# Dao-AILab/flash-attention

Measured on AMD Instinct MI355X. Metric: attention_fwd_tflops, higher is better.
Workload: dtype bf16; 1 GPU; BASELINE config 3: B=4 H=32 S=4096 D=128 bf16 causal, forward (flash_attn_func path, fa_fwd via C ABI); batch=4, heads=32, seqlen=4096, head_dim=128, causal=True, parallelism=replicas x1

## Files before the change

flash-attention_amd/csrc/fa_fwd_w64.hip:

```cpp
#include <cstdio>
#include <cstdlib>
#include <type_traits>

#include "fa_device.h"
#include "fa_kernel_params.h"
#include "fa_launch.h"
#include "fa_fwd_w64_regs.h"
#define FA_W64_CLOB FA_W64_ACC_CLOBBERS
#include "fa_w64_asm.h"


#define FA_W64_AH 3
#define FA_W64_KDMA_G0 0
#define FA_W64_KDMA_GS 2
#define FA_W64_VDMA_G0 1
#define FA_W64_VDMA_GS 2

namespace fa {

template <int D> FA_DEVINL constexpr int k_swz_w(int row) { return D == 128 ? (row & 15) : ((row >> 1) & 7); }
template <int D> FA_DEVINL constexpr int v_swz_w(int row) { return D == 128 ? (row & 3) : ((row >> 1) & 1); }

#define FA_W64_MFMA(E_) (std::is_same<E_, __bf16>::value ? "v_mfma_f32_32x32x16_bf16" : "v_mfma_f32_32x32x16_f16")
constexpr int W64_Q_BASE = 128;
template <typename E, int F> FA_DEVINL void mfma_s_first(f32x16& d, u32x4 a, const f32x16& c) {
  if constexpr (std::is_same<E, __bf16>::value)
    asm volatile("v_mfma_f32_32x32x16_bf16 %0, %1, a[%c3:%c4], %2" : "=&v"(d) : "v"(a), "v"(c), "i"(W64_Q_BASE + 4 * F), "i"(W64_Q_BASE + 4 * F + 3) : FA_W64_ACC_CLOBBERS);
  else
    asm volatile("v_mfma_f32_32x32x16_f16 %0, %1, a[%c3:%c4], %2" : "=&v"(d) : "v"(a), "v"(c), "i"(W64_Q_BASE + 4 * F), "i"(W64_Q_BASE + 4 * F + 3) : FA_W64_ACC_CLOBBERS);
}
template <typename E, int F> FA_DEVINL void mfma_s_acc(f32x16& d, u32x4 a) {
  if constexpr (std::is_same<E, __bf16>::value)
    asm volatile("v_mfma_f32_32x32x16_bf16 %0, %1, a[%c2:%c3], %0" : "+v"(d) : "v"(a), "i"(W64_Q_BASE + 4 * F), "i"(W64_Q_BASE + 4 * F + 3) : FA_W64_ACC_CLOBBERS);
  else
    asm volatile("v_mfma_f32_32x32x16_f16 %0, %1, a[%c2:%c3], %0" : "+v"(d) : "v"(a), "i"(W64_Q_BASE + 4 * F), "i"(W64_Q_BASE + 4 * F + 3) : FA_W64_ACC_CLOBBERS);
}
template <typename E, int T> FA_DEVINL void mfma_o_acc(u32x4 a, u32x4 b) {
  if constexpr (std::is_same<E, __bf16>::value)
    asm volatile("v_mfma_f32_32x32x16_bf16 a[%c2:%c3], %0, %1, a[%c2:%c3]" : : "v"(a), "v"(b), "i"(16 * T), "i"(16 * T + 15) : FA_W64_ACC_CLOBBERS);
  else
    asm volatile("v_mfma_f32_32x32x16_f16 a[%c2:%c3], %0, %1, a[%c2:%c3]" : : "v"(a), "v"(b), "i"(16 * T), "i"(16 * T + 15) : FA_W64_ACC_CLOBBERS);
}
template <typename E, int D, int FEAT = 0, bool PAGED = false>
__global__ void __launch_bounds__(256, 1) fa_fwd_w64_kernel(const FwdK p) {
  constexpr bool ALIBI = FEAT == FEAT_ALIBI;
  static_assert(!PAGED || FEAT == 0, "the paged variant serves plain attention");
  constexpr bool SOFTCAP = FEAT == FEAT_CAP;
  constexpr bool DROP = FEAT == FEAT_DROP;
  constexpr bool DESC = ALIBI;
  static_assert(FEAT == 0 || FEAT == FEAT_ALIBI || FEAT == FEAT_CAP || FEAT == FEAT_DROP, "feature variants of this schedule: none, causal ALiBi, softcap, dropout");
  using T = ElemTraits<E>;
  using V8 = typename T::v8;
  constexpr int NW = 4, QB = 2, BM = NW * 64, BN = 64, CPR = D / 8;
  constexpr int ROW_BYTES = D * 2;
  constexpr int TILE_BYTES = BN * ROW_BYTES;
  constexpr int KS = D / 16;
  constexpr int DB = D / 32;
  static_assert(D == 64 || D == 128, "head dims built natively: 64, 128");
  constexpr float kLn2 = 0.6931471805599453f;

  extern __shared__ __attribute__((aligned(16))) char smem[];
  char FA_LDS* lds = (char FA_LDS*)smem;
  constexpr int STAGE_BYTES = BM * (ROW_BYTES + 16);
  constexpr int Q_OFF = (4 * TILE_BYTES > STAGE_BYTES ? 4 * TILE_BYTES : STAGE_BYTES + 1023) / 1024 * 1024;

  const int tid = threadIdx.x;
  const int lane = tid & 63;
  const int wave = __builtin_amdgcn_readfirstlane(tid >> 6);
  const int hi = lane >> 5, qi = lane & 31;

  const int d_row = lane / CPR, d_pc = lane % CPR;
  constexpr int RPD = 1024 / ROW_BYTES;

  struct Blk { int b, h, m_block, sq, sk; int64_t q_row0, k_row0, q_boff, k_boff, v_boff, o_boff; };
  const int n_virtual = p.persist_total > 0 ? p.persist_total : (int)gridDim.x;
  const bool snake = p.persist_total > 0 && p.wr >= 0 && p.unit_size > 1 && ((int)(gridDim.x / 8) % p.unit_size) == 0;
  auto decode_id = [&](int vb, int round, Blk& k) __attribute__((always_inline)) -> bool {
    if (vb >= n_virtual) return false;
    if (p.work_list) {
      if (!work_list_item(p.work_list, vb, p.h, p.h_k, k.b, k.h, k.m_block)) return false;
    } else {
      int bid = vb;
      if (snake && (round & 1)) {
        const int slot = vb / 8, item = slot % p.unit_size;
        bid = vb + 8 * (p.unit_size - 1 - 2 * item);
      }
      const int w = xcd_interleave(bid, p.n_units, p.unit_size, p.unit_hpx);
      if (w < 0) return false;
      const int bh = w / p.nmb;
      const int mbr = w - bh * p.nmb;
      k.m_block = (p.wr >= 0) ? (p.nmb - 1 - mbr) : mbr;
      k.b = bh / p.h;
      k.h = bh - k.b * p.h;
    }
    return true;
  };
  auto fill_blk = [&](Blk& k) __attribute__((always_inline)) -> bool {
    k.sq = p.sq; k.sk = p.sk; k.q_row0 = 0; k.k_row0 = 0;
    const int bkv = p.kv_batch_idx ? p.kv_batch_idx[k.b] : k.b;
    k.q_boff = (int64_t)k.b * p.q_bs; k.k_boff = (int64_t)bkv * p.k_bs; k.v_boff = (int64_t)bkv * p.v_bs; k.o_boff = (int64_t)k.b * p.o_bs;
    if (p.cu_q) { const int c0 = p.cu_q[k.b]; k.sq = p.cu_q[k.b + 1] - c0; k.q_row0 = c0; k.q_boff = 0; k.o_boff = 0; }
    if (p.seqused_q) k.sq = min(k.sq, p.seqused_q[k.b]);
    if (p.cu_k) { const int c0 = p.cu_k[k.b]; k.sk = p.cu_k[k.b + 1] - c0; k.k_row0 = c0; k.k_boff = 0; k.v_boff = 0; }
    if (p.seqused_k) k.sk = min(p.seqused_k[k.b] + p.seqused_add, (p.cu_k && !PAGED) ? k.sk : p.sk);
    if (p.leftpad_k) {
      const int lp = p.leftpad_k[k.b];
      k.sk = max(0, k.sk - lp);
      k.k_row0 += lp;
    }
    if constexpr (PAGED) { k.k_boff = 0; k.v_boff = 0; k.k_row0 = 0; }
    return k.m_block * BM < k.sq;
  };
  constexpr int QDMA = (BM * ROW_BYTES) / 1024 / NW;
  auto q_srd_of = [&](const Blk& k) __attribute__((always_inline)) {
    const E* base = (const E*)p.q + k.q_boff + (k.q_row0 + (int64_t)k.m_block * BM) * p.q_rs + (int64_t)k.h * p.q_hs;
    const int rows = min(BM, k.sq - k.m_block * BM);
    const unsigned long long a = (unsigned long long)base;
// ... 87 lines not shown
    const unsigned long long a = (unsigned long long)base;
    const unsigned lo = __builtin_amdgcn_readfirstlane((unsigned)a);
    const unsigned hi16 = __builtin_amdgcn_readfirstlane((unsigned)(a >> 32)) & 0xffffu;
    const unsigned long long bytes = sk > 0 ? ((unsigned long long)(sk - 1) * (unsigned long long)row_stride + D) * 2ull : 0ull;
    const unsigned nrec = __builtin_amdgcn_readfirstlane((unsigned)(bytes > 0xffffffffull ? 0xffffffffull : bytes));
    u32x4 s = {lo, hi16, nrec, 0x00020000u};
    return s;
  };
  const u32x4 k_srd = make_srd(kp, p.k_rs), v_srd = make_srd(vp, p.v_rs);
  const u32x4 null_srd = {k_srd[0], k_srd[1], 0u, k_srd[3]};
  const int pg_tpp = __builtin_amdgcn_readfirstlane(PAGED ? p.page_size / BN : 1);
  const int pg_last = __builtin_amdgcn_readfirstlane(sk > 0 ? (sk - 1) / max(p.page_size, 1) : 0);
  const int* __restrict__ pg_table = p.block_table + (PAGED ? (int64_t)__builtin_amdgcn_readfirstlane(b) * p.block_table_bs : 0);
  auto page_entry = [&](int page) __attribute__((always_inline)) {
    const int pc = min(max(page, 0), pg_last);
    return __builtin_amdgcn_readfirstlane(pg_table[pc]);
  };
  const unsigned pg_bytes_k = (unsigned)__builtin_amdgcn_readfirstlane((int)(unsigned)(p.k_bs * 2)), pg_bytes_v = (unsigned)__builtin_amdgcn_readfirstlane((int)(unsigned)(p.v_bs * 2));
  const unsigned tl_bytes_k = (unsigned)__builtin_amdgcn_readfirstlane((int)(unsigned)(BN * p.k_rs * 2)), tl_bytes_v = (unsigned)__builtin_amdgcn_readfirstlane((int)(unsigned)(BN * p.v_rs * 2));
  auto uniform64 = [](const void* ptr) __attribute__((always_inline)) {
    const unsigned long long a = (unsigned long long)ptr;
    const unsigned lo = (unsigned)__builtin_amdgcn_readfirstlane((int)(unsigned)a), hi = (unsigned)__builtin_amdgcn_readfirstlane((int)(unsigned)(a >> 32));
    return ((unsigned long long)hi << 32) | (unsigned long long)lo;
  };
  const unsigned long long pg_base_k = uniform64(kp), pg_base_v = uniform64(vp);
  auto tile_srd = [&](auto isvc, int blk, int tin, int n) __attribute__((always_inline)) {
    constexpr bool ISV = decltype(isvc)::value != 0;
    const unsigned rs = (unsigned)(ISV ? p.v_rs : p.k_rs);
    const int rows = (n >= 0) ? min(BN, sk - n * BN) : 0;
    const unsigned long long a = (ISV ? pg_base_v : pg_base_k) + (unsigned long long)(unsigned)blk * (unsigned long long)(ISV ? pg_bytes_v : pg_bytes_k) + (unsigned long long)((unsigned)tin * (ISV ? tl_bytes_v : tl_bytes_k));
    const unsigned nrec = rows > 0 ? ((unsigned)(rows - 1) * rs + (unsigned)D) * 2u : 0u;
    u32x4 sd = {(unsigned)a, (unsigned)(a >> 32) & 0xffffu, nrec, 0x00020000u};
    return sd;
  };
  auto dma_pieces = [&](const u32x4& srd, const unsigned (&vo)[DPW], unsigned lds_dst) __attribute__((always_inline)) {
    unsigned keep;
    const unsigned dst = __builtin_amdgcn_readfirstlane(lds_dst);
    if constexpr (DPW == 4) {
      asm volatile("s_mov_b32 %0, m0\n\ts_mov_b32 m0, %5\n\ts_nop 0\n\t"
                   "buffer_load_dwordx4 %1, %6, 0 offen lds\n\t"
                   "buffer_load_dwordx4 %2, %6, 0 offen offset:1024 lds\n\t"
                   "buffer_load_dwordx4 %3, %6, 0 offen offset:2048 lds\n\t"
                   "buffer_load_dwordx4 %4, %6, 0 offen offset:3072 lds\n\t"
                   "s_mov_b32 m0, %0"
                   : "=&s"(keep) : "v"(vo[0]), "v"(vo[1]), "v"(vo[2]), "v"(vo[3]), "s"(dst), "s"(srd) : "memory");
    } else {
      asm volatile("s_mov_b32 %0, m0\n\ts_mov_b32 m0, %3\n\ts_nop 0\n\t"
                   "buffer_load_dwordx4 %1, %4, 0 offen lds\n\t"
                   "buffer_load_dwordx4 %2, %4, 0 offen offset:1024 lds\n\t"
                   "s_mov_b32 m0, %0"
                   : "=&s"(keep) : "v"(vo[0]), "v"(vo[DPW - 1]), "s"(dst), "s"(srd) : "memory");
    }
  };
  auto dma_tile = [&](auto isvc, int buf, int t) __attribute__((always_inline)) {
    constexpr bool ISV = decltype(isvc)::value != 0;
    const bool real = t >= 0 && t < n_tiles;
    const int64_t rs = ISV ? p.v_rs : p.k_rs;
    const unsigned lds_dst = (unsigned)((ISV ? 2 + buf : buf) * TILE_BYTES + wave * DPW * 1024);
    if constexpr (PAGED) {
      const int n = n_min + t, page = max(n, 0) / pg_tpp;
      const u32x4 sd = real ? tile_srd(isvc, page_entry(page), max(n, 0) - page * pg_tpp, n) : null_srd;
      dma_pieces(sd, ISV ? voff_l : koff_l, lds_dst);
      return;
    }
    const unsigned toff = real ? (unsigned)(n_min + t) * (unsigned)(BN * 2) * (unsigned)rs : 0u;
    unsigned vo[DPW];
#pragma unroll
    for (int i = 0; i < DPW; ++i) vo[i] = (ISV ? voff_l[i] : koff_l[i]) + toff;
    dma_pieces(real ? (ISV ? v_srd : k_srd) : null_srd, vo, lds_dst);
  };

  __syncthreads();
  if (q_in_lds != vb) dma_q(q_srd_of(blk));
  if (n_tiles > 0) dma_tile(ICw<0>{}, 0, tile_of(0));
  if (q_in_lds != vb) {
    if (n_tiles > 0) { if constexpr (DPW == 4) asm volatile("s_waitcnt vmcnt(4)" ::: "memory"); else asm volatile("s_waitcnt vmcnt(2)" ::: "memory"); }
    else lds_dma_wait_all();
  }
  {
    const float cq = SOFTCAP ? p.scale * 2.885390081777927f / p.softcap : p.scale_log2;
    u32x4 qraw[QB][KS];
#pragma unroll
    for (int qb = 0; qb < QB; ++qb)
#pragma unroll
      for (int ks = 0; ks < KS; ++ks) {
        const int qbase = Q_OFF + (wave * 64 + qb * 32 + qi) * ROW_BYTES + ((hi ^ k_swz_w<D>(qi)) << 4);
        qraw[qb][ks] = *(const u32x4 FA_LDS*)(unsigned long)(unsigned)(qbase ^ (ks << 5));
      }
    auto load_q = [&](auto qbc, auto ksc) __attribute__((always_inline)) {
      constexpr int qb = decltype(qbc)::value, ks = decltype(ksc)::value;
      const V8 raw = bitcast_u32x4<V8>(qraw[qb][ks]);
      V8 sc;
#pragma unroll
      for (int j = 0; j < 8; j += 2) {
        typedef __attribute__((ext_vector_type(2))) float f32x2;
        f32x2 pr = {(float)raw[j], (float)raw[j + 1]};
        pr *= f32x2{cq, cq};
        sc[j] = (E)pr[0]; sc[j + 1] = (E)pr[1];
      }
      acc_write_frag<W64_Q_BASE + 4 * (qb * KS + ks)>(__builtin_bit_cast(u32x4, sc));
    };
    auto load_q_all = [&](auto qbc) __attribute__((always_inline)) {
      load_q(qbc, ICw<0>{}); load_q(qbc, ICw<1>{}); load_q(qbc, ICw<2>{}); load_q(qbc, ICw<3>{});
      if constexpr (KS == 8) { load_q(qbc, ICw<4>{}); load_q(qbc, ICw<5>{}); load_q(qbc, ICw<6>{}); load_q(qbc, ICw<7>{}); }
    };
    load_q_all(ICw<0>{});
    if (n_tiles > 0) dma_tile(ICw<1>{}, 1, -1);
    load_q_all(ICw<1>{});
  }
  lds_dma_wait_all();
  __syncthreads();
  u32x4 qn_srd = null_srd;
  int qn_done = QDMA, qn_per_iter = QDMA;
  {
    q_in_lds = -1;
    if (nxt_id_ok && fill_blk(nxt)) {
      asm volatile("s_waitcnt lgkmcnt(0)" ::: "memory");
      qn_srd = q_srd_of(nxt); qn_done = 0;
      qn_per_iter = n_tiles >= QDMA ? 1 : n_tiles >= QDMA / 2 ? 2 : n_tiles >= QDMA / 4 ? 4 : QDMA;
      if (n_tiles == 0) { dma_q(qn_srd); lds_dma_wait_all(); qn_done = QDMA; }
      q_in_lds = vb + (int)gridDim.x;
    }
  }
  auto q_trickle = [&]() __attribute__((always_inline)) {
    if (qn_done < QDMA) {
#pragma unroll 1
      for (int j = 0; j < qn_per_iter; ++j) dma_q_piece(qn_srd, qn_done + j);
      qn_done += qn_per_iter;
    }
  };

  const int kbase = qi * ROW_BYTES + ((hi ^ k_swz_w<D>(qi)) << 4);
  const int tr_i = lane & 15, tr_half = (lane >> 4) & 1;
  const int tr_rr = tr_i >> 2, tr_cc = tr_i & 3;
  const int vbase = (4 * hi + tr_rr) * ROW_BYTES + (v_swz_w<D>(tr_rr) << 6) + tr_half * 32 + tr_cc * 8;
  int ka[KS], va[DB];
#pragma unroll
  for (int ks = 0; ks < KS; ++ks) ka[ks] = kbase ^ (ks << 5);
#pragma unroll
  for (int db = 0; db < DB; ++db) va[db] = vbase ^ (db << 6);

  {
    u32x4 zf = {0u, 0u, 0u, 0u};
    asm volatile("" : "+v"(zf));
    acc_zero_tuples_mfma<0>(zf, std::make_integer_sequence<int, 2 * DB>{});
  }
  float m_run[QB], l_run[QB][2], o_lag[QB];
  float thr_l[QB];
  float capc = 0.f, cap_m2c = 0.f, capoff[QB] = {0.f, 0.f};
  if constexpr (SOFTCAP) {
    capc = __builtin_bit_cast(float, __builtin_amdgcn_readfirstlane(__builtin_bit_cast(int, p.softcap * 1.4426950408889634f)));
    cap_m2c = -2.f * capc;
    capoff[0] = capc; capoff[1] = capc;
  }
  unsigned drop_kr[7] = {0u, 0u, 0u, 0u, 0u, 0u, 0u}, drop_thr = 255u, drop_row[QB] = {0u, 0u};
  if constexpr (DROP) {
    const unsigned k0_ = (unsigned)__builtin_amdgcn_readfirstlane((int)drop_bh_key(p.rng, b * p.h + h));
#pragma unroll
    for (int r = 0; r < 7; ++r) drop_kr[r] = k0_ + (unsigned)r * 0x9E3779B9u;
    drop_thr = (unsigned)__builtin_amdgcn_readfirstlane((int)p.drop_thr8);
#pragma unroll
    for (int qb = 0; qb < QB; ++qb) drop_row[qb] = (unsigned)(w_row0 + 32 * qb + qi);
  }
  constexpr float kCapTiny = 7.888609052210118e-31f;
  unsigned long long lag_mask = 0ull;
  f32x16 negm[QB];
  int arel[QB] = {0, 0};
  if constexpr (ALIBI) {
#pragma unroll
    for (int qb = 0; qb < QB; ++qb) arel[qb] = 4 * hi - (w_row0 + 32 * qb + qi) - shift;
  }
  const float ainc = slope2 * 32.f;
  f32x16 sA[QB], sB[QB];
  u32x4 pfA[QB][2], pfB[QB][2];
#pragma unroll
  for (int qb = 0; qb < QB; ++qb) {
    m_run[qb] = -INFINITY; l_run[qb][0] = 0.f; l_run[qb][1] = 0.f; o_lag[qb] = 1.f; thr_l[qb] = -INFINITY;
#pragma unroll
    for (int r = 0; r < 16; ++r) { negm[qb][r] = ALIBI ? slope2 * (float)(arel[qb] + step_key(0) + acc_row(r, 0)) : 0.f; sA[qb][r] = -INFINITY; sB[qb][r] = -INFINITY; }
#pragma unroll
    for (int t = 0; t < 2; ++t) { pfA[qb][t] = u32x4{0u, 0u, 0u, 0u}; pfB[qb][t] = u32x4{0u, 0u, 0u, 0u}; }
  }

  auto rescale = [&](auto qbc, bool grow, float tmax, f32x16& s_nxt) __attribute__((always_inline)) {
    constexpr int qb = decltype(qbc)::value;
    const float m_base = (m_run[qb] == -INFINITY) ? 0.f : m_run[qb];
    const float m_upd = grow ? (tmax + m_base) : m_run[qb];
    const float m_safe = (m_upd == -INFINITY) ? 0.f : m_upd;
    const float alpha = (grow && m_run[qb] != -INFINITY) ? fast_exp2(m_run[qb] - m_safe) : 1.f;
    const float delta = m_safe - m_base;
    m_run[qb] = m_upd;
    thr_l[qb] = grow ? thr : thr_l[qb];
    l_run[qb][0] *= alpha;
// ... 23 lines not shown
      lag_mask = __builtin_amdgcn_ballot_w64(o_lag[0] != 1.f || o_lag[1] != 1.f) != 0ull ? ~0ull : 0ull;
    }
  };
  auto set_mask = [&](int i_step) __attribute__((always_inline)) {
    const int k0m = step_key(i_step);
    float ninf = -INFINITY;
    asm volatile("" : "+v"(ninf));
    static_for<QB>([&](auto mqc) __attribute__((always_inline)) {
      constexpr int mq = decltype(mqc)::value;
      float nb = (SOFTCAP || m_run[mq] == -INFINITY) ? 0.f : -m_run[mq];
      const int rel_hi = min(lim_hi[mq] - k0m - 4 * hi, 31), rel_lo = max(lim_lo[mq] - k0m - 4 * hi, 0);
      const unsigned ones = (rel_hi - rel_lo >= 31) ? 0xffffffffu : ((2u << ((rel_hi - rel_lo) & 31)) - 1u);
      unsigned bits = (rel_hi >= rel_lo) ? (ones << (rel_lo & 31)) : 0u;
      if constexpr (ALIBI) nb += slope2 * (float)(arel[mq] + k0m);
      asm volatile("" : "+v"(nb), "+v"(bits));
#pragma unroll
      for (int r = 0; r < 16; r += 4) {
        float n0 = negm[mq][r], n1 = negm[mq][r + 1], n2 = negm[mq][r + 2], n3 = negm[mq][r + 3];
        unsigned t0, t1;
        if constexpr (ALIBI) {
          const float v0 = nb + slope2 * (float)acc_row(r, 0), v1 = nb + slope2 * (float)acc_row(r + 1, 0);
          const float v2 = nb + slope2 * (float)acc_row(r + 2, 0), v3 = nb + slope2 * (float)acc_row(r + 3, 0);
          asm volatile("v_bfe_i32 %4, %6, %c11, 1\n\tv_bfe_i32 %5, %6, %c12, 1\n\tv_bfi_b32 %0, %4, %7, %15\n\tv_bfi_b32 %1, %5, %8, %15\n\t"
                       "v_bfe_i32 %4, %6, %c13, 1\n\tv_bfe_i32 %5, %6, %c14, 1\n\tv_bfi_b32 %2, %4, %9, %15\n\tv_bfi_b32 %3, %5, %10, %15"
                       : "+v"(n0), "+v"(n1), "+v"(n2), "+v"(n3), "=&v"(t0), "=&v"(t1)
                       : "v"(bits), "v"(v0), "v"(v1), "v"(v2), "v"(v3), "i"(acc_row(r, 0)), "i"(acc_row(r + 1, 0)), "i"(acc_row(r + 2, 0)), "i"(acc_row(r + 3, 0)),
                         "v"(ninf));
        } else {
          asm volatile("v_bfe_i32 %4, %6, %c9, 1\n\tv_bfe_i32 %5, %6, %c10, 1\n\tv_bfi_b32 %0, %4, %7, %8\n\tv_bfi_b32 %1, %5, %7, %8\n\t"
                       "v_bfe_i32 %4, %6, %c11, 1\n\tv_bfe_i32 %5, %6, %c12, 1\n\tv_bfi_b32 %2, %4, %7, %8\n\tv_bfi_b32 %3, %5, %7, %8"
                       : "+v"(n0), "+v"(n1), "+v"(n2), "+v"(n3), "=&v"(t0), "=&v"(t1)
                       : "v"(bits), "v"(nb), "v"(ninf), "i"(acc_row(r, 0)), "i"(acc_row(r + 1, 0)), "i"(acc_row(r + 2, 0)), "i"(acc_row(r + 3, 0)));
        }
        negm[mq][r] = n0; negm[mq][r + 1] = n1; negm[mq][r + 2] = n2; negm[mq][r + 3] = n3;
      }
    });
  };
  auto clear_mask = [&](int i_next) __attribute__((always_inline)) {
    static_for<QB>([&](auto mqc) __attribute__((always_inline)) {
      constexpr int mq = decltype(mqc)::value;
      float nb = (SOFTCAP || m_run[mq] == -INFINITY) ? 0.f : -m_run[mq];
      if constexpr (ALIBI) nb += slope2 * (float)(arel[mq] + step_key(i_next));
      asm volatile("" : "+v"(nb));
#pragma unroll
      for (int r = 0; r < 16; ++r) {
        float nv = negm[mq][r];
        float val = nb;
        if constexpr (ALIBI) val = nb + slope2 * (float)acc_row(r, 0);
        asm volatile("v_mov_b32 %0, %1" : "+v"(nv) : "v"(val));
        negm[mq][r] = nv;
      }
    });
  };
  auto fast_step = [&](auto halfc, auto parc, f32x16 (&s_cur)[QB], f32x16 (&s_nxt)[QB],
                       const u32x4 (&pf_prev)[QB][2], u32x4 (&pf_cur)[QB][2], const u32x4& dma_srd, const unsigned (&dma_off)[DPW],
                       unsigned dma_toff, unsigned dma_dst, u32x4 (&kfr)[FA_W64_AH + 1], int drop_k0q = 0, auto modec = ICw<0>{}) __attribute__((always_inline)) {
    constexpr int half = decltype(halfc)::value, par = decltype(parc)::value;
    constexpr int MODE = decltype(modec)::value;
    constexpr bool DO_QK = MODE <= 2, DO_P = MODE == 0 || MODE == 2 || MODE == 3, DO_PV = MODE == 0 || MODE >= 3;
    constexpr int QKG = 2 * KS, PVG = 4 * DB, NG = QKG + PVG;
    auto drop_gap = [](int G, int r) constexpr { return ((7 * G + r) * (NG - 2)) / 56; };
    constexpr bool drop_in_time = [&]() constexpr {
      constexpr int cpg = 16 / PVG > 0 ? 16 / PVG : 1;
      for (int G = 0; G < 8; ++G) if (drop_gap(G, 6) >= QKG + (2 * G) / cpg) return false;
      return true;
    }();
    static_assert(!DROP || drop_in_time, "a Philox word is finished before its first element is packed");
    unsigned ph_c0[8], ph_c1[8];
    constexpr int KOFF = par * TILE_BYTES + half * 32 * ROW_BYTES;
    constexpr int VOFF = (2 + (par ^ 1)) * TILE_BYTES + half * 32 * ROW_BYTES;
    constexpr int AH = FA_W64_AH, RING = AH + 1;
    constexpr int NF = KS + 2 * DB;
    static_assert(RING == FA_W64_AH + 1, "the K fragment ring is the caller's (carried from a first step to its second step)");
    s16x4 vlo[RING], vhi[RING];
    auto rd_frag = [&](int f) __attribute__((always_inline)) {
      if (f < KS) {
        if constexpr (DO_QK) kfr[f % RING] = *(const u32x4 FA_LDS*)(unsigned long)(unsigned)(ka[f] + KOFF);
      } else if (f < NF && DO_PV) {
        const int op = f - KS;
        const char FA_LDS* a0 = (const char FA_LDS*)(unsigned long)(unsigned)(va[op % DB] + VOFF + (16 * (op / DB)) * ROW_BYTES);
        vlo[f % RING] = lds_read_tr16(a0);
        vhi[f % RING] = lds_read_tr16(a0 + 8 * ROW_BYTES);
      }
    };
    auto el_end = [](int x) constexpr { return SOFTCAP ? 32 : x <= QKG ? (24 * x) / QKG : (24 + ((x - QKG) * 16) / PVG > 32 ? 32 : 24 + ((x - QKG) * 16) / PVG); };
    float pe[QB][16];
    auto cap_a = [](int x) constexpr {
      if (x <= 0) return 0;
      if (x <= QKG) return (20 * x) / QKG;
      const int n = 20 + ((x - QKG) * 12 + (PVG - 3)) / (PVG - 2);
      return n > 32 ? 32 : n;
    };
    static_assert(!SOFTCAP || cap_a(NG - 2) == 32, "every element's last stage inside the step");
    float cap_a1[32], cap_d[32], cap_arg[32], cap_g[QB] = {0.f, 0.f}, cap_gt[QB] = {-INFINITY, -INFINITY};
    float tmax[QB] = {-INFINITY, -INFINITY}, tcopy[QB] = {0.f, 0.f};
    constexpr int UPG = PVG >= 16 ? 1 : 2;
    auto tree_g0 = [](int mq) constexpr { return 1 + mq; };
    auto hm_gap = [&](int mq) constexpr { return tree_g0(mq) + 8 / UPG; };
    if constexpr (half != 1) {
#pragma unroll
      for (int f = 0; f < AH; ++f) rd_frag(f);
    }
    __builtin_amdgcn_sched_barrier(0);
    static_for<NG>([&](auto xc) __attribute__((always_inline)) {
      constexpr int x = decltype(xc)::value;
      constexpr int f = x / 2, qb = x & 1;
      if constexpr (qb == 0) rd_frag(f + AH);
      if constexpr (qb == 0 && (f & 1) == 0 && f + 1 < NF) {
        constexpr auto ops = [](int g) constexpr { return g < KS ? (DO_QK ? 1 : 0) : g < NF ? (DO_PV ? 2 : 0) : 0; };
        constexpr int out = [&]() constexpr { int n = 0; for (int g = f + 2; g <= f + AH; ++g) n += ops(g); return n; }();
        if constexpr (f < KS ? DO_QK : DO_PV) __builtin_amdgcn_s_waitcnt(0xC07F | (out << 8));
      }
      if constexpr (x < QKG ? !DO_QK : !DO_PV) {
        if constexpr (x == QKG && DO_QK) mfma_drain_acc();
      } else if constexpr (x < QKG) {
        if constexpr (f == 0) mfma_s_first<E, qb * KS>(s_nxt[qb], kfr[f % RING], negm[qb]);
        else mfma_s_acc<E, qb * KS + f>(s_nxt[qb], kfr[f % RING]);
      } else {
        constexpr int op = f - KS;
        const u32x4 vf = __builtin_bit_cast(u32x4, combine_tr<V8>(vlo[f % RING], vhi[f % RING]));
        mfma_o_acc<E, qb * DB + op % DB>(vf, pf_prev[qb][op / DB]);
      }
      constexpr int G0 = half == 0 ? FA_W64_KDMA_G0 : FA_W64_VDMA_G0, GS = half == 0 ? FA_W64_KDMA_GS : FA_W64_VDMA_GS;
      if constexpr (x >= G0 && (x - G0) % GS == 0 && (x - G0) / GS < DPW) {
        constexpr int pc = (x - G0) / GS;
        if constexpr (pc == 0)
          asm volatile("s_mov_b32 m0, %1\n\ts_nop 0\n\tbuffer_load_dwordx4 %0, %2, %3 offen lds" : : "v"(dma_off[pc]), "s"(dma_dst), "s"(dma_srd), "s"(dma_toff) : "memory");
        else
          asm volatile("buffer_load_dwordx4 %0, %1, %3 offen offset:%c2 lds" : : "v"(dma_off[pc]), "s"(dma_srd), "i"(1024 * pc), "s"(dma_toff) : "memory");
      }
      if constexpr (ALIBI) {
        constexpr auto ab_end = [](int g) constexpr { return g < 4 ? 0 : (((g - 3) * 32 + (NG - 5)) / (NG - 4) > 32 ? 32 : ((g - 3) * 32 + (NG - 5)) / (NG - 4)); };
        const float step_add = (half == 1 && DESC) ? -3.f * ainc : ainc;
#pragma unroll
        for (int e = ab_end(x); e < ab_end(x + 1); ++e) {
          float nv = negm[e >> 4][e & 15];
          asm volatile("v_add_f32 %0, %0, %1" : "+v"(nv) : "v"(step_add));
          negm[e >> 4][e & 15] = nv;
        }
      }
      if constexpr (DROP) {
#pragma unroll
        for (int G = 0; G < 8; ++G)
#pragma unroll
          for (int r = 0; r < 7; ++r)
            if (drop_gap(G, r) == x) {
              if (r == 0) { ph_c0[G] = (unsigned)(drop_k0q + 2 * (G & 3)) + (unsigned)hi; ph_c1[G] = drop_row[G >> 2]; }
              const unsigned mh = __umulhi(0xD256D193u, ph_c0[G]), ml = 0xD256D193u * ph_c0[G];
              unsigned x3;
              asm("v_bitop3_b32 %0, %1, %2, %3 bitop3:0x96" : "=v"(x3) : "v"(mh), "s"(drop_kr[r]), "v"(ph_c1[G]));
              ph_c0[G] = x3;
              ph_c1[G] = ml;
            }
      }
      if constexpr (SOFTCAP) {
#pragma unroll
        for (int e = cap_a(x - 2); e < cap_a(x - 1); ++e) {
          const int eq = e >> 4, r = e & 15;
          pe[eq][r] = fast_exp2(cap_arg[e]);
          l_run[eq][r & 1] += pe[eq][r];
        }
#pragma unroll
        for (int e = cap_a(x - 1); e < cap_a(x); ++e) cap_arg[e] = __builtin_fmaf(__builtin_amdgcn_rcpf(cap_d[e]), cap_m2c, cap_a1[e]);
#pragma unroll
// ... 8 lines not shown
        const int eq = e >> 4, r = e & 15;
        pe[eq][r] = fast_exp2(s_cur[eq][r]);
        l_run[eq][r & 1] += pe[eq][r];
      }
      if constexpr (x >= QKG) {
        constexpr int y = x - QKG;
        constexpr int CPG = 16 / PVG > 0 ? 16 / PVG : 1;
#pragma unroll
        for (int c = (DO_P ? y * CPG : 16); c < (y + 1) * CPG && c < 16; ++c) {
          const int j = c >> 2, m = c & 3, cq = j >> 1, t = j & 1;
          using V2 = __attribute__((ext_vector_type(2))) E;
          V2 pr;
          float pv0 = pe[cq][8 * t + 2 * m], pv1 = pe[cq][8 * t + 2 * m + 1];
          if constexpr (DROP) {
            const int r0 = 8 * t + 2 * m;
            const unsigned w = ph_c0[4 * cq + (r0 >> 2)];
            pv0 = (((w >> (8 * (r0 & 3))) & 0xffu) > drop_thr) ? 0.f : pv0;
            pv1 = (((w >> (8 * ((r0 + 1) & 3))) & 0xffu) > drop_thr) ? 0.f : pv1;
          }
          pr[0] = (E)pv0;
          pr[1] = (E)pv1;
          unsigned pw = __builtin_bit_cast(unsigned, pr);
          asm volatile("" : "+v"(pw));
          pf_cur[cq][t][m] = pw;
        }
#pragma unroll
        for (int mq = (DO_QK ? 0 : QB); mq < QB; ++mq) {
          const int g0 = tree_g0(mq);
          if (y >= g0 && y < g0 + 8 / UPG) {
#pragma unroll
            for (int u = (y - g0) * UPG; u < (y - g0 + 1) * UPG; ++u)
              if (u == 7 && UPG == 1) {
                float t_in = tmax[mq], t_out, t_cp;
                asm volatile("v_max_f32 %0, %2, %3\n\tv_mov_b32 %1, %0" : "=&v"(t_out), "=v"(t_cp) : "v"(t_in), "v"(s_nxt[mq][15]));
                tmax[mq] = t_out; tcopy[mq] = t_cp;
              } else
              tmax[mq] = u == 0 ? vmax3(s_nxt[mq][0], s_nxt[mq][1], s_nxt[mq][2])
                                : u < 7 ? vmax3(tmax[mq], s_nxt[mq][2 * u + 1], s_nxt[mq][2 * u + 2]) : vmax2(tmax[mq], s_nxt[mq][15]);
          }
          if (y == hm_gap(mq) - 1 && UPG != 1) asm volatile("v_mov_b32 %0, %1" : "=v"(tcopy[mq]) : "v"(tmax[mq]));
          if (y == hm_gap(mq)) {
            if constexpr (!DO_PV) asm volatile("s_nop 1\n\tv_permlane32_swap_b32 %0, %1\n\tv_max_f32 %0, %0, %1" : "+v"(tmax[mq]), "+v"(tcopy[mq]));
            else asm volatile("v_permlane32_swap_b32 %0, %1\n\tv_max_f32 %0, %0, %1" : "+v"(tmax[mq]), "+v"(tcopy[mq]));
          }
          if constexpr (SOFTCAP) {
            constexpr int last = PVG - 1;
            const int g1 = hm_gap(mq) + 1 < last ? hm_gap(mq) + 1 : last, g2 = hm_gap(mq) + 2 < last ? hm_gap(mq) + 2 : last, g3 = hm_gap(mq) + 3 < last ? hm_gap(mq) + 3 : last;
            if (y == g1) cap_g[mq] = fast_exp2(tmax[mq]) + 1.f;
            if (y == g2) cap_g[mq] = __builtin_fmaf(__builtin_amdgcn_rcpf(cap_g[mq]), cap_m2c, capoff[mq]);
            if (y == g3) cap_gt[mq] = __builtin_fmaf(tmax[mq], kCapTiny, cap_g[mq]);
          }
        }
      }
      if constexpr (half == 0 && x >= NG - AH && DO_QK) {
        constexpr int fn = x - (NG - AH);
        kfr[fn % RING] = *(const u32x4 FA_LDS*)(unsigned long)(unsigned)(ka[fn] + par * TILE_BYTES + 32 * ROW_BYTES);
      }
      __builtin_amdgcn_sched_barrier(0);
    });
#pragma unroll
    for (int mq = 0; mq < QB; ++mq)
      if (hm_gap(mq) >= PVG && DO_QK) tmax[mq] = vhalf_max(tmax[mq]);
    static_assert(!SOFTCAP || QB + 8 / UPG < PVG - 1, "softcap: the capped maximum is made inside the gaps");
    if constexpr (SOFTCAP) { tmax[0] = cap_gt[0]; tmax[1] = cap_gt[1]; }
    if constexpr (MODE != 4) decide_and_rescale(tmax, s_nxt);
  };

  int u_first = n_tiles + 1, u_last = n_tiles, p_lo = n_tiles + 1, p_hi = n_tiles;
  if (wave_valid && n_tiles > 0) {
    const int a_lo = max(0, (w_kmin - key_base) >> 5);
    const int a_hi = min(n_steps - 1, (w_kmax - key_base) >> 5);
    if (a_hi >= a_lo) {
      u_first = a_lo >> 1; u_last = min(n_tiles, (a_hi + 2) >> 1);
      const int f_lo = max(0, (w_full_lo - key_base + 31) >> 5);
      const int f_hi = (w_full_hi - 31 - key_base) >> 5;
      p_lo = max(u_first, (f_lo + 1) >> 1);
      p_hi = min(u_last, (f_hi - 1) >> 1);
      if constexpr (DESC) {
        const int t_lo = a_lo >> 1, t_hi = a_hi >> 1, pl_t = (f_lo + 1) >> 1, ph_t = (f_hi - 1) >> 1;
        u_first = n_tiles - 1 - t_hi; u_last = n_tiles - t_lo;
        p_lo = max(u_first, n_tiles - 1 - ph_t);
        p_hi = min(u_last, n_tiles - 1 - pl_t);
      }
      if (p_hi < p_lo) { p_lo = u_last + 1; p_hi = u_last; }
    }
  }
  u_first = __builtin_amdgcn_readfirstlane(u_first); u_last = __builtin_amdgcn_readfirstlane(u_last);
  const unsigned wave_dst = (unsigned)(wave * DPW * 1024);
  auto iter_end = [&]() __attribute__((always_inline)) {
    lds_dma_wait_all();
    __syncthreads();
  };
  const int m_lo = __builtin_amdgcn_readfirstlane(p_lo), m_hi = __builtin_amdgcn_readfirstlane(p_hi);
  const unsigned step_k = (unsigned)(BN * 2) * (unsigned)p.k_rs, step_v = (unsigned)(BN * 2) * (unsigned)p.v_rs;
  const int nmin_s = __builtin_amdgcn_readfirstlane(n_min), nts_s = __builtin_amdgcn_readfirstlane(n_tiles);
  int pg_blk_k = 0, pg_tin_k = 0, pg_blk_v = 0, pg_tin_v = 0, pg_page_n = 0, pg_tin_n = 0;
  auto pg_enter = [&](int u) __attribute__((always_inline)) {
    if constexpr (PAGED) {
      const int nv = n_min + u, nk = nv + 1, nn = nv + 2;
      pg_tin_v = nv % pg_tpp; pg_blk_v = page_entry(nv / pg_tpp);
      pg_tin_k = nk % pg_tpp; pg_blk_k = page_entry(nk / pg_tpp);
      pg_page_n = nn / pg_tpp; pg_tin_n = nn - pg_page_n * pg_tpp;
    }
  };
  auto step_pair = [&](auto parc, int u, auto pmc) __attribute__((always_inline)) {
    constexpr int par = decltype(parc)::value, PM = decltype(pmc)::value;
    using M0 = ICw<(PM == 1 ? 1 : PM == 2 ? 3 : 0)>; using M1 = ICw<(PM == 1 ? 2 : PM == 2 ? 4 : 0)>;
    q_trickle();
    u32x4 kring[FA_W64_AH + 1];
    const int us = __builtin_amdgcn_readfirstlane(u);
    unsigned dst_k = (unsigned)((par ^ 1) * TILE_BYTES) + wave_dst, dst_v = (unsigned)((2 + par) * TILE_BYTES) + wave_dst;
    unsigned tk_ = (unsigned)(nmin_s + (DESC ? nts_s - 2 - us : us + 1)) * step_k, tv_ = (unsigned)(nmin_s + (DESC ? nts_s - 1 - us : us)) * step_v;
    int im32 = ((us - m_lo) | (m_hi - us)) >> 31;
    dst_k = __builtin_amdgcn_readfirstlane(dst_k); dst_v = __builtin_amdgcn_readfirstlane(dst_v);
    im32 = __builtin_amdgcn_readfirstlane(im32);
    u32x4 srd_k = k_srd, srd_v = v_srd;
    if constexpr (PAGED) {
      const int bk = __builtin_amdgcn_readfirstlane(pg_blk_k), tk = __builtin_amdgcn_readfirstlane(pg_tin_k);
      const int bv = __builtin_amdgcn_readfirstlane(pg_blk_v), tv = __builtin_amdgcn_readfirstlane(pg_tin_v);
      const int pn = __builtin_amdgcn_readfirstlane(pg_page_n), tn = __builtin_amdgcn_readfirstlane(pg_tin_n);
      srd_k = tile_srd(ICw<0>{}, bk, tk, nmin_s + us + 1);
      srd_v = tile_srd(ICw<1>{}, bv, tv, nmin_s + us);
      tk_ = 0u; tv_ = 0u;
      pg_blk_v = bk; pg_tin_v = tk;
      pg_blk_k = page_entry(pn); pg_tin_k = tn;
      const bool wrap = tn + 1 == pg_tpp;
      pg_tin_n = wrap ? 0 : tn + 1;
      pg_page_n = wrap ? pn + 1 : pn;
    }
    asm volatile("" : "+s"(tk_), "+s"(tv_), "+s"(dst_k), "+s"(dst_v), "+s"(im32));
    auto masked = [&]() __attribute__((always_inline)) { int c = im32; asm volatile("" : "+s"(c)); return c != 0; };
    if constexpr (PM != 2) { if (__builtin_expect(masked(), 0)) set_mask(2 * u); }
    fast_step(ICw<0>{}, parc, sA, sB, pfA, pfB, srd_k, koff_l, tk_, dst_k, kring, DROP ? step_key(2 * us - 1) >> 2 : 0, M0{});
    if constexpr (PM != 2) { if (__builtin_expect(masked(), 0)) set_mask(2 * u + 1); }
    fast_step(ICw<1>{}, parc, sB, sA, pfB, pfA, srd_v, voff_l, tv_, dst_v, kring, DROP ? step_key(2 * us) >> 2 : 0, M1{});
    if constexpr (PM != 2) { if (__builtin_expect(masked(), 0)) clear_mask(2 * u + 2); }
    iter_end();
  };
  auto idle_iter = [&](int u) __attribute__((always_inline)) {
    q_trickle();
    dma_tile(ICw<0>{}, (u & 1) ^ 1, tile_of(u + 1)); dma_tile(ICw<1>{}, u & 1, tile_of(u));
    iter_end();
  };
  if (n_tiles > 0) {
    const bool active = u_first <= u_last;
    const int ua = active ? (u_first & ~1) : n_tiles + 1;
    int u = 0;
#pragma unroll 1
    for (; u < ua; ++u) idle_iter(u);
    if (active) {
      pg_enter(u);
      if constexpr (ALIBI) { if (u > 0) clear_mask(2 * u); }
      if constexpr (FEAT == 0) {
        step_pair(ICw<0>{}, u, ICw<1>{}); ++u;
#pragma unroll 1
        for (;;) {
          if (u >= u_last) break;
          step_pair(ICw<1>{}, u, ICw<0>{}); ++u;
          if (u >= u_last) break;
          step_pair(ICw<0>{}, u, ICw<0>{}); ++u;
        }
        if (u & 1) step_pair(ICw<1>{}, u, ICw<2>{}); else step_pair(ICw<0>{}, u, ICw<2>{});
        ++u;
      } else {
#pragma unroll 1
        for (;;) {
          step_pair(ICw<0>{}, u, ICw<0>{}); ++u;
          if (u > u_last) break;
          step_pair(ICw<1>{}, u, ICw<0>{}); ++u;
          if (u > u_last) break;
        }
      }
    }
#pragma unroll 1
    for (; u <= n_tiles; ++u) idle_iter(u);
  }

  if (wave_valid) {
  mfma_drain_acc();
  u32x4 o_srd;
  {
    const int rows = min(BM, sq - m0);
    const unsigned long long a = (unsigned long long)(op + (int64_t)m0 * p.o_rs);
    const unsigned lo = __builtin_amdgcn_readfirstlane((unsigned)a);
    const unsigned hi16 = __builtin_amdgcn_readfirstlane((unsigned)(a >> 32)) & 0xffffu;
    const unsigned nr = __builtin_amdgcn_readfirstlane((unsigned)(((unsigned long long)(rows - 1) * (unsigned long long)p.o_rs + D) * 2ull));
    o_srd = u32x4{lo, hi16, nr, 0x00020000u};
  }
  static_for<QB>([&](auto qbc) __attribute__((always_inline)) {
    constexpr int qb = decltype(qbc)::value;
    f32x16 o_v[DB];
    static_for<DB>([&](auto dbc) __attribute__((always_inline)) {
      constexpr int db = decltype(dbc)::value;
      acc_read_tuple<16 * (qb * DB + db)>(o_v[db]);
#pragma unroll
      for (int r = 0; r < 16; ++r) o_v[db][r] = o_v[db][r];
    });
    const float l_tot = half_sum(l_run[qb][0] + l_run[qb][1]);
    const bool dead = (l_tot == 0.f) || (l_tot != l_tot);
    const float inv = (dead ? 1.f : 1.f / l_tot) * o_lag[qb] * (DROP ? p.rp_keep : 1.f);
    const int row0 = w_row0 + 32 * qb;
    if (row0 < sq) {
      {
        using V4 = typename T::v4;
        constexpr int RS = ROW_BYTES + 16, RPI = 64 / CPR;
        char FA_LDS* stage = lds + (wave * 64 + qb * 32) * RS;
#pragma unroll
        for (int db = 0; db < DB; ++db)
#pragma unroll
          for (int g = 0; g < 4; ++g) {
            V4 ov;
#pragma unroll
            for (int jj = 0; jj < 4; ++jj) ov[jj] = (E)(o_v[db][4 * g + jj] * inv);
            *reinterpret_cast<V4 FA_LDS*>(stage + qi * RS + (32 * db + 8 * g + 4 * hi) * 2) = ov;
          }
        unsigned lane_off = (unsigned)(((wave * 64 + lane / CPR) * (int)p.o_rs + (lane % CPR) * 8) * 2);
        asm volatile("" : "+v"(lane_off));
#pragma unroll
        for (int i = 0; i < 32 / RPI; ++i) {
          const u32x4 x = *reinterpret_cast<const u32x4 FA_LDS*>(stage + (i * RPI + lane / CPR) * RS + (lane % CPR) * 16);
          const unsigned soff = __builtin_amdgcn_readfirstlane((unsigned)((qb * 32 + i * RPI) * (int)p.o_rs * 2));
          asm volatile("buffer_store_dwordx4 %0, %1, %2, %3 offen" : : "v"(x), "v"(lane_off), "s"(o_srd), "s"(soff) : "memory");
        }
        asm volatile("s_waitcnt lgkmcnt(0)" ::: "memory");
      }
      const int my_row = row0 + qi;
      if (my_row < sq && hi == 0) lsep[my_row] = dead ? INFINITY : (m_run[qb] * kLn2 + __logf(l_tot));
    }
  });
  }
  }
}

template <typename E, int D, int FEAT = 0, bool PAGED = false>
static int launch_fwd_w64_t(const FwdK& p, hipStream_t stream) {
  constexpr int STAGE = 256 * (D * 2 + 16);
  constexpr int smem = ((4 * 64 * D * 2 > STAGE ? 4 * 64 * D * 2 : STAGE + 1023) / 1024 * 1024) + 256 * D * 2;
  auto kern = fa_fwd_w64_kernel<E, D, FEAT, PAGED>;
  static std::atomic<unsigned long long> attr_mask{0};
  if (ensure_dyn_lds(attr_mask, (const void*)kern, smem, true) != 0) return -1;
  const long long total = p.work_list ? (long long)p.work_bound * p.h : units_grid(p.n_units, p.unit_size);
  if (total <= 0) return 0;
  FwdK pp = p;
  long long grid = total;
  const int cus = device_cu_count();
  const bool balanced = p.wr < 0 || (p.unit_size > 1 && (cus / 8) % p.unit_size == 0);
  if (!p.work_list && cus >= 8 && total > cus && balanced && knobs().w64_persist != 0) {
    grid = cus / 8 * 8;
    pp.persist_total = (int)total;
  }
  hipLaunchKernelGGL(kern, dim3((unsigned)grid), dim3(256), smem, stream, pp);
  if (hipGetLastError() != hipSuccess) return -1;
  LastSchedule& ls = last_schedule();
  ls.fwd_kernel = 3; ls.fwd_nw = 4; ls.fwd_feat = FEAT; ls.fwd_splits = 1; ls.fwd_list = p.work_list != nullptr; ls.d = D;
  ls.bf16 = std::is_same<E, __bf16>::value;
  if (FEAT) snprintf(ls.name, sizeof(ls.name), "fa::fa_fwd_w64_kernel<%s,%d,%s>", ls.bf16 ? "bf16" : "f16", D, FEAT == FEAT_CAP ? "softcap" : FEAT == FEAT_DROP ? "dropout" : "alibi");
  else if (PAGED) snprintf(ls.name, sizeof(ls.name), "fa::fa_fwd_w64_kernel<%s,%d,paged>", ls.bf16 ? "bf16" : "f16", D);
  else snprintf(ls.name, sizeof(ls.name), "fa::fa_fwd_w64_kernel<%s,%d>", ls.bf16 ? "bf16" : "f16", D);
  return 0;
}

#ifndef FA_W64_PART
#define FA_W64_PART 0
#endif
int launch_fwd_w64_bf16(const FwdK& p, int d, hipStream_t stream);
int launch_fwd_w64_f16(const FwdK& p, int d, hipStream_t stream);
#if FA_W64_PART != 1
int launch_fwd_w64_f16(const FwdK& p, int d, hipStream_t stream) {
  if (p.rng) {
    if (d == 128) return launch_fwd_w64_t<_Float16, 128, FEAT_DROP>(p, stream);
    if (d == 64) return launch_fwd_w64_t<_Float16, 64, FEAT_DROP>(p, stream);
    return -2;
  }
  if (p.softcap > 0.f) {
    if (d == 128) return launch_fwd_w64_t<_Float16, 128, FEAT_CAP>(p, stream);
    if (d == 64) return launch_fwd_w64_t<_Float16, 64, FEAT_CAP>(p, stream);
    return -2;
  }
  if (p.alibi) {
    if (d == 128) return launch_fwd_w64_t<_Float16, 128, FEAT_ALIBI>(p, stream);
    if (d == 64) return launch_fwd_w64_t<_Float16, 64, FEAT_ALIBI>(p, stream);
    return -2;
  }
  if (p.block_table) {
    if (d == 128) return launch_fwd_w64_t<_Float16, 128, 0, true>(p, stream);
    if (d == 64) return launch_fwd_w64_t<_Float16, 64, 0, true>(p, stream);
    return -2;
  }
  if (d == 128) return launch_fwd_w64_t<_Float16, 128>(p, stream);
  if (d == 64) return launch_fwd_w64_t<_Float16, 64>(p, stream);
// ... 45 lines not shown
```

Baseline: 1099 TFLOP/s.

## Triple-buffer K/V LDS tiles to deepen DMA prefetch by one tile

Grows the K and V LDS ring from two to three slots each, so DMA for tile u+2 (K) and u+1 (V) is issued while tile u is computed. The per-iteration wait now leaves the newest tile's loads outstanding instead of draining all of them. The K fragment ring is hoisted to persist across step pairs, and the next step's first K fragments are prefetched at the end of each half. This removes exposed global-load latency but raises LDS use to six tiles, which may cut occupancy, and it adds modulo-3 slot arithmetic plus a new three-phase steady loop.

```diff
diff --git a/flash-attention_amd/csrc/fa_fwd_w64.hip b/flash-attention_amd/csrc/fa_fwd_w64.hip
--- a/flash-attention_amd/csrc/fa_fwd_w64.hip
+++ b/flash-attention_amd/csrc/fa_fwd_w64.hip
@@ -62,7 +62,8 @@
   extern __shared__ __attribute__((aligned(16))) char smem[];
   char FA_LDS* lds = (char FA_LDS*)smem;
   constexpr int STAGE_BYTES = BM * (ROW_BYTES + 16);
-  constexpr int Q_OFF = (4 * TILE_BYTES > STAGE_BYTES ? 4 * TILE_BYTES : STAGE_BYTES + 1023) / 1024 * 1024;
+  constexpr int Q_OFF = (6 * TILE_BYTES > STAGE_BYTES ? 6 * TILE_BYTES : STAGE_BYTES + 1023) / 1024 * 1024;
+  constexpr int V_BASE = 3 * TILE_BYTES;
 
   const int tid = threadIdx.x;
   const int lane = tid & 63;
@@ -256,11 +257,11 @@
                    : "=&s"(keep) : "v"(vo[0]), "v"(vo[DPW - 1]), "s"(dst), "s"(srd) : "memory");
     }
   };
-  auto dma_tile = [&](auto isvc, int buf, int t) __attribute__((always_inline)) {
+  auto dma_tile = [&](auto isvc, int slot, int t) __attribute__((always_inline)) {
     constexpr bool ISV = decltype(isvc)::value != 0;
     const bool real = t >= 0 && t < n_tiles;
     const int64_t rs = ISV ? p.v_rs : p.k_rs;
-    const unsigned lds_dst = (unsigned)((ISV ? 2 + buf : buf) * TILE_BYTES + wave * DPW * 1024);
+    const unsigned lds_dst = (unsigned)((ISV ? 3 + slot : slot) * TILE_BYTES + wave * DPW * 1024);
     if constexpr (PAGED) {
       const int n = n_min + t, page = max(n, 0) / pg_tpp;
       const u32x4 sd = real ? tile_srd(isvc, page_entry(page), max(n, 0) - page * pg_tpp, n) : null_srd;
@@ -309,10 +310,11 @@
       if constexpr (KS == 8) { load_q(qbc, ICw<4>{}); load_q(qbc, ICw<5>{}); load_q(qbc, ICw<6>{}); load_q(qbc, ICw<7>{}); }
     };
     load_q_all(ICw<0>{});
-    if (n_tiles > 0) dma_tile(ICw<1>{}, 1, -1);
+    if (n_tiles > 0) { dma_tile(ICw<1>{}, 2, -1); dma_tile(ICw<0>{}, 1, tile_of(1)); }
     load_q_all(ICw<1>{});
-  }
-  lds_dma_wait_all();
+    if (n_tiles > 0) dma_tile(ICw<1>{}, 0, tile_of(0));
+  }
+  if (n_tiles > 0) { if constexpr (DPW == 4) asm volatile("s_waitcnt vmcnt(4)" ::: "memory"); else asm volatile("s_waitcnt vmcnt(2)" ::: "memory"); }
   __syncthreads();
   u32x4 qn_srd = null_srd;
   int qn_done = QDMA, qn_per_iter = QDMA;
@@ -342,7 +344,7 @@
 #pragma unroll
   for (int ks = 0; ks < KS; ++ks) ka[ks] = kbase ^ (ks << 5);
 #pragma unroll
-  for (int db = 0; db < DB; ++db) va[db] = vbase ^ (db << 6);
+  for (int db = 0; db < DB; ++db) va[db] = (vbase ^ (db << 6)) + V_BASE;
 
   {
     u32x4 zf = {0u, 0u, 0u, 0u};
@@ -472,10 +474,13 @@
       }
     });
   };
-  auto fast_step = [&](auto halfc, auto parc, f32x16 (&s_cur)[QB], f32x16 (&s_nxt)[QB],
+  auto fast_step = [&](auto halfc, auto slotc, f32x16 (&s_cur)[QB], f32x16 (&s_nxt)[QB],
                        const u32x4 (&pf_prev)[QB][2], u32x4 (&pf_cur)[QB][2], const u32x4& dma_srd, const unsigned (&dma_off)[DPW],
-                       unsigned dma_toff, unsigned dma_dst, u32x4 (&kfr)[FA_W64_AH + 1], int drop_k0q = 0, auto modec = ICw<0>{}) __attribute__((always_inline)) {
-    constexpr int half = decltype(halfc)::value, par = decltype(parc)::value;
+                       unsigned dma_toff, unsigned dma_dst, u32x4 (&kfr)[FA_W64_AH + 1], int drop_k0q = 0, auto modec = ICw<0>{},
+                       int rk = 0, int rv = 0, int rc = 0) __attribute__((always_inline)) {
+    constexpr int half = decltype(halfc)::value;
+    constexpr bool RT = decltype(slotc)::value == 3;
+    constexpr int slot = RT ? 0 : decltype(slotc)::value;
     constexpr int MODE = decltype(modec)::value;
     constexpr bool DO_QK = MODE <= 2, DO_P = MODE == 0 || MODE == 2 || MODE == 3, DO_PV = MODE == 0 || MODE >= 3;
     constexpr int QKG = 2 * KS, PVG = 4 * DB, NG = QKG + PVG;
@@ -487,18 +492,19 @@
     }();
     static_assert(!DROP || drop_in_time, "a Philox word is finished before its first element is packed");
     unsigned ph_c0[8], ph_c1[8];
-    constexpr int KOFF = par * TILE_BYTES + half * 32 * ROW_BYTES;
-    constexpr int VOFF = (2 + (par ^ 1)) * TILE_BYTES + half * 32 * ROW_BYTES;
+    constexpr int KOFF = (RT ? 0 : slot * TILE_BYTES) + half * 32 * ROW_BYTES;
+    constexpr int VOFF = (RT ? 0 : ((slot + 2) % 3) * TILE_BYTES) + half * 32 * ROW_BYTES;
+    constexpr int COFF = half == 0 ? (RT ? 0 : slot * TILE_BYTES) + 32 * ROW_BYTES : (RT ? 0 : ((slot + 1) % 3) * TILE_BYTES);
     constexpr int AH = FA_W64_AH, RING = AH + 1;
     constexpr int NF = KS + 2 * DB;
     static_assert(RING == FA_W64_AH + 1, "the K fragment ring is the caller's (carried from a first step to its second step)");
     s16x4 vlo[RING], vhi[RING];
     auto rd_frag = [&](int f) __attribute__((always_inline)) {
       if (f < KS) {
-        if constexpr (DO_QK) kfr[f % RING] = *(const u32x4 FA_LDS*)(unsigned long)(unsigned)(ka[f] + KOFF);
+        if constexpr (DO_QK) kfr[f % RING] = *(const u32x4 FA_LDS*)(unsigned long)(unsigned)(ka[f] + rk + KOFF);
       } else if (f < NF && DO_PV) {
         const int op = f - KS;
-        const char FA_LDS* a0 = (const char FA_LDS*)(unsigned long)(unsigned)(va[op % DB] + VOFF + (16 * (op / DB)) * ROW_BYTES);
+        const char FA_LDS* a0 = (const char FA_LDS*)(unsigned long)(unsigned)(va[op % DB] + rv + VOFF + (16 * (op / DB)) * ROW_BYTES);
         vlo[f % RING] = lds_read_tr16(a0);
         vhi[f % RING] = lds_read_tr16(a0 + 8 * ROW_BYTES);
       }
@@ -517,10 +523,6 @@
     constexpr int UPG = PVG >= 16 ? 1 : 2;
     auto tree_g0 = [](int mq) constexpr { return 1 + mq; };
     auto hm_gap = [&](int mq) constexpr { return tree_g0(mq) + 8 / UPG; };
-    if constexpr (half != 1) {
-#pragma unroll
-      for (int f = 0; f < AH; ++f) rd_frag(f);
-    }
     __builtin_amdgcn_sched_barrier(0);
     static_for<NG>([&](auto xc) __attribute__((always_inline)) {
       constexpr int x = decltype(xc)::value;
@@ -529,7 +531,7 @@
       if constexpr (qb == 0 && (f & 1) == 0 && f + 1 < NF) {
         constexpr auto ops = [](int g) constexpr { return g < KS ? (DO_QK ? 1 : 0) : g < NF ? (DO_PV ? 2 : 0) : 0; };
         constexpr int out = [&]() constexpr { int n = 0; for (int g = f + 2; g <= f + AH; ++g) n += ops(g); return n; }();
-        if constexpr (f < KS ? DO_QK : DO_PV) __builtin_amdgcn_s_waitcnt(0xC07F | (out << 8));
+        if constexpr ((f < KS ? DO_QK : DO_PV) && !(half == 0 && f == 0)) __builtin_amdgcn_s_waitcnt(0xC07F | (out << 8));
       }
       if constexpr (x < QKG ? !DO_QK : !DO_PV) {
         if constexpr (x == QKG && DO_QK) mfma_drain_acc();
@@ -644,9 +646,9 @@
           }
         }
       }
-      if constexpr (half == 0 && x >= NG - AH && DO_QK) {
+      if constexpr (x >= NG - AH && DO_QK) {
         constexpr int fn = x - (NG - AH);
-        kfr[fn % RING] = *(const u32x4 FA_LDS*)(unsigned long)(unsigned)(ka[fn] + par * TILE_BYTES + 32 * ROW_BYTES);
+        kfr[fn % RING] = *(const u32x4 FA_LDS*)(unsigned long)(unsigned)(ka[fn] + (half == 0 ? rk : rc) + COFF);
       }
       __builtin_amdgcn_sched_barrier(0);
     });
@@ -679,8 +681,9 @@
   }
   u_first = __builtin_amdgcn_readfirstlane(u_first); u_last = __builtin_amdgcn_readfirstlane(u_last);
   const unsigned wave_dst = (unsigned)(wave * DPW * 1024);
+  u32x4 kring[FA_W64_AH + 1];
   auto iter_end = [&]() __attribute__((always_inline)) {
-    lds_dma_wait_all();
+    if constexpr (DPW == 4) asm volatile("s_waitcnt vmcnt(4)" ::: "memory"); else asm volatile("s_waitcnt vmcnt(2)" ::: "memory");
     __syncthreads();
   };
   const int m_lo = __builtin_amdgcn_readfirstlane(p_lo), m_hi = __builtin_amdgcn_readfirstlane(p_hi);
@@ -689,20 +692,20 @@
   int pg_blk_k = 0, pg_tin_k = 0, pg_blk_v = 0, pg_tin_v = 0, pg_page_n = 0, pg_tin_n = 0;
   auto pg_enter = [&](int u) __attribute__((always_inline)) {
     if constexpr (PAGED) {
-      const int nv = n_min + u, nk = nv + 1, nn = nv + 2;
+      const int nv = n_min + u + 1, nk = nv + 1, nn = nv + 2;
       pg_tin_v = nv % pg_tpp; pg_blk_v = page_entry(nv / pg_tpp);
       pg_tin_k = nk % pg_tpp; pg_blk_k = page_entry(nk / pg_tpp);
       pg_page_n = nn / pg_tpp; pg_tin_n = nn - pg_page_n * pg_tpp;
     }
   };
-  auto step_pair = [&](auto parc, int u, auto pmc) __attribute__((always_inline)) {
-    constexpr int par = decltype(parc)::value, PM = decltype(pmc)::value;
+  auto step_pair = [&](auto slotc, int u, auto pmc) __attribute__((always_inline)) {
+    constexpr int SLOT = decltype(slotc)::value, PM = decltype(pmc)::value;
     using M0 = ICw<(PM == 1 ? 1 : PM == 2 ? 3 : 0)>; using M1 = ICw<(PM == 1 ? 2 : PM == 2 ? 4 : 0)>;
     q_trickle();
-    u32x4 kring[FA_W64_AH + 1];
     const int us = __builtin_amdgcn_readfirstlane(u);
-    unsigned dst_k = (unsigned)((par ^ 1) * TILE_BYTES) + wave_dst, dst_v = (unsigned)((2 + par) * TILE_BYTES) + wave_dst;
-    unsigned tk_ = (unsigned)(nmin_s + (DESC ? nts_s - 2 - us : us + 1)) * step_k, tv_ = (unsigned)(nmin_s + (DESC ? nts_s - 1 - us : us)) * step_v;
+    const int srt = SLOT == 3 ? us % 3 : SLOT;
+    unsigned dst_k = (unsigned)(((srt + 2) % 3) * TILE_BYTES) + wave_dst, dst_v = (unsigned)((3 + (srt + 1) % 3) * TILE_BYTES) + wave_dst;
+    unsigned tk_ = (unsigned)(nmin_s + (DESC ? nts_s - 3 - us : us + 2)) * step_k, tv_ = (unsigned)(nmin_s + (DESC ? nts_s - 2 - us : us + 1)) * step_v;
     int im32 = ((us - m_lo) | (m_hi - us)) >> 31;
     dst_k = __builtin_amdgcn_readfirstlane(dst_k); dst_v = __builtin_amdgcn_readfirstlane(dst_v);
     im32 = __builtin_amdgcn_readfirstlane(im32);
@@ -711,8 +714,8 @@
       const int bk = __builtin_amdgcn_readfirstlane(pg_blk_k), tk = __builtin_amdgcn_readfirstlane(pg_tin_k);
       const int bv = __builtin_amdgcn_readfirstlane(pg_blk_v), tv = __builtin_amdgcn_readfirstlane(pg_tin_v);
       const int pn = __builtin_amdgcn_readfirstlane(pg_page_n), tn = __builtin_amdgcn_readfirstlane(pg_tin_n);
-      srd_k = tile_srd(ICw<0>{}, bk, tk, nmin_s + us + 1);
-      srd_v = tile_srd(ICw<1>{}, bv, tv, nmin_s + us);
+      srd_k = tile_srd(ICw<0>{}, bk, tk, nmin_s + us + 2);
+      srd_v = tile_srd(ICw<1>{}, bv, tv, nmin_s + us + 1);
       tk_ = 0u; tv_ = 0u;
       pg_blk_v = bk; pg_tin_v = tk;
       pg_blk_k = page_entry(pn); pg_tin_k = tn;
@@ -722,17 +725,35 @@
     }
     asm volatile("" : "+s"(tk_), "+s"(tv_), "+s"(dst_k), "+s"(dst_v), "+s"(im32));
     auto masked = [&]() __attribute__((always_inline)) { int c = im32; asm volatile("" : "+s"(c)); return c != 0; };
+    const int rk = SLOT == 3 ? srt * TILE_BYTES : 0, rv = SLOT == 3 ? ((srt + 2) % 3) * TILE_BYTES : 0, rc = SLOT == 3 ? ((srt + 1) % 3) * TILE_BYTES : 0;
     if constexpr (PM != 2) { if (__builtin_expect(masked(), 0)) set_mask(2 * u); }
-    fast_step(ICw<0>{}, parc, sA, sB, pfA, pfB, srd_k, koff_l, tk_, dst_k, kring, DROP ? step_key(2 * us - 1) >> 2 : 0, M0{});
+    fast_step(ICw<0>{}, slotc, sA, sB, pfA, pfB, srd_k, koff_l, tk_, dst_k, kring, DROP ? step_key(2 * us - 1) >> 2 : 0, M0{}, rk, rv, rc);
     if constexpr (PM != 2) { if (__builtin_expect(masked(), 0)) set_mask(2 * u + 1); }
-    fast_step(ICw<1>{}, parc, sB, sA, pfB, pfA, srd_v, voff_l, tv_, dst_v, kring, DROP ? step_key(2 * us) >> 2 : 0, M1{});
+    fast_step(ICw<1>{}, slotc, sB, sA, pfB, pfA, srd_v, voff_l, tv_, dst_v, kring, DROP ? step_key(2 * us) >> 2 : 0, M1{}, rk, rv, rc);
     if constexpr (PM != 2) { if (__builtin_expect(masked(), 0)) clear_mask(2 * u + 2); }
     iter_end();
   };
   auto idle_iter = [&](int u) __attribute__((always_inline)) {
     q_trickle();
-    dma_tile(ICw<0>{}, (u & 1) ^ 1, tile_of(u + 1)); dma_tile(ICw<1>{}, u & 1, tile_of(u));
+    const int us = __builtin_amdgcn_readfirstlane(u);
+    dma_tile(ICw<0>{}, (us + 2) % 3, tile_of(us + 2)); dma_tile(ICw<1>{}, (us + 1) % 3, tile_of(us + 1));
     iter_end();
+  };
+  auto kring_fill = [&](int u) __attribute__((always_inline)) {
+    const int rk = (__builtin_amdgcn_readfirstlane(u) % 3) * TILE_BYTES;
+#pragma unroll
+    for (int f = 0; f < FA_W64_AH; ++f) kring[f] = *(const u32x4 FA_LDS*)(unsigned long)(unsigned)(ka[f] + rk);
+  };
+  auto steady = [&](int& u, int u_end) __attribute__((always_inline)) {
+    int ph = __builtin_amdgcn_readfirstlane(u) % 3;
+#pragma unroll 1
+    for (;;) {
+      if (ph == 0) { if (u >= u_end) break; step_pair(ICw<0>{}, u, ICw<0>{}); ++u; }
+      if (ph <= 1) { if (u >= u_end) break; step_pair(ICw<1>{}, u, ICw<0>{}); ++u; }
+      if (u >= u_end) break;
+      step_pair(ICw<2>{}, u, ICw<0>{}); ++u;
+      ph = 0;
+    }
   };
   if (n_tiles > 0) {
     const bool active = u_first <= u_last;
@@ -743,29 +764,19 @@
     if (active) {
       pg_enter(u);
       if constexpr (ALIBI) { if (u > 0) clear_mask(2 * u); }
+      kring_fill(u);
       if constexpr (FEAT == 0) {
-        step_pair(ICw<0>{}, u, ICw<1>{}); ++u;
-#pragma unroll 1
-        for (;;) {
-          if (u >= u_last) break;
-          step_pair(ICw<1>{}, u, ICw<0>{}); ++u;
-          if (u >= u_last) break;
-          step_pair(ICw<0>{}, u, ICw<0>{}); ++u;
-        }
-        if (u & 1) step_pair(ICw<1>{}, u, ICw<2>{}); else step_pair(ICw<0>{}, u, ICw<2>{});
-        ++u;
+        step_pair(ICw<3>{}, u, ICw<1>{}); ++u;
+        steady(u, u_last);
+        step_pair(ICw<3>{}, u, ICw<2>{}); ++u;
       } else {
-#pragma unroll 1
-        for (;;) {
-          step_pair(ICw<0>{}, u, ICw<0>{}); ++u;
-          if (u > u_last) break;
-          step_pair(ICw<1>{}, u, ICw<0>{}); ++u;
-          if (u > u_last) break;
-        }
+        steady(u, u_last + 1);
       }
     }
 #pragma unroll 1
     for (; u <= n_tiles; ++u) idle_iter(u);
+    lds_dma_wait_all();
+    __syncthreads();
   }
 
   if (wave_valid) {
@@ -827,7 +838,7 @@
 template <typename E, int D, int FEAT = 0, bool PAGED = false>
 static int launch_fwd_w64_t(const FwdK& p, hipStream_t stream) {
   constexpr int STAGE = 256 * (D * 2 + 16);
-  constexpr int smem = ((4 * 64 * D * 2 > STAGE ? 4 * 64 * D * 2 : STAGE + 1023) / 1024 * 1024) + 256 * D * 2;
+  constexpr int smem = ((6 * 64 * D * 2 > STAGE ? 6 * 64 * D * 2 : STAGE + 1023) / 1024 * 1024) + 256 * D * 2;
   auto kern = fa_fwd_w64_kernel<E, D, FEAT, PAGED>;
   static std::atomic<unsigned long long> attr_mask{0};
   if (ensure_dyn_lds(attr_mask, (const void*)kern, smem, true) != 0) return -1;
```

After: 1090 TFLOP/s (median of 2 runs). About the same (-0.8%).
